# CESSProject/DeOSS

Measured on AMD Instinct MI355X. Metric: device-resident GiB/s hashed to Merkle root; 1/2/4/8 MI355X scaling, higher is better.
Workload: dtype u32; 1 GPU; BASELINE configs[1]: 1 object of 8 GiB (8589934592 B) in 1 chunk-range shard(s) of 8 GiB, chunk 33554432 B (256 leaves); object_bytes=8589934592, chunk=33554432, leaves=256, parallelism=single GPU

## Files before the change

### deoss_amd/csrc/merkle_capi.hip

```cpp
#include <hip/hip_runtime.h>
#include <rccl/rccl.h>

#include <algorithm>
#include <atomic>
#include <chrono>
#include <condition_variable>
#include <deque>
#include <cerrno>
#include <cstdarg>
#include <cstdlib>
#include <cstdio>
#include <cstring>
#include <functional>
#include <map>
#include <memory>
#include <future>
#include <mutex>
#include <string>
#include <thread>
#include <type_traits>
#include <vector>

#include "deoss_merkle.h"
#include "merkle_kernels.hpp"
// ... 200 lines not shown
                std::unique_lock<std::mutex> lk(mu);
                cv.wait(lk, [&] { return stop || !q.empty(); });
                if (q.empty()) return;
                it = q.front();
                q.pop_front();
                active++;
            }
            (void)hipSetDevice(it.dev);
            (void)hipGetLastError();
            if (it.pinned) host_release(it.p);
            else dev_release(it.dev, it.p);
            {
                std::lock_guard<std::mutex> lk(mu);
                active--;
            }
            idle.notify_all();
        }
    }
    void drain() {
        std::unique_lock<std::mutex> lk(mu);
        idle.wait(lk, [&] { return q.empty() && active == 0; });
    }
    void finish() {
        {
            std::lock_guard<std::mutex> lk(mu);
            stop = true;
        }
        cv.notify_one();
        if (th.joinable()) th.join();
    }
    ~Reaper() { finish(); }
};

void reaper_put(Reaper* r, int dev, void* p, bool pinned) { r->put(dev, p, pinned); }
void reaper_drain(Reaper* r) { r->drain(); }

void par_copy(const std::vector<dm_copy::CopyItem>& items) { dm_copy::CopyPool::get().run(items); }

struct StreamKit {
    static constexpr int kEvents = 10, kSlots = 4;
    hipStream_t copy = nullptr;
    hipStream_t code = nullptr, comp[2] = {nullptr, nullptr};
    hipEvent_t ev[kEvents] = {};
    PinnedBuf slot[kSlots];
    PinnedBuf tabs;
    uint64_t tabs_used = 0;
};

struct Dev {
    int id = 0;
    int cus = 256;
    hipStream_t stream = nullptr;
    hipStream_t copy = nullptr;
    DevBuf data, nodes_a, nodes_b, leaves, tab_addr, tab_len, tab_first, tab_ids, root, gather;
    DevBuf proof_paths, proof_bits, proof_roots;
    DevBuf aes_win;
    PinnedBuf stage[2];
    PinnedBuf htab;
    uint64_t htab_used = 0;
    hipEvent_t ev_done = nullptr;
    hipEvent_t ev_copy[2] = {nullptr, nullptr}, ev_step[2] = {nullptr, nullptr}, ev_htab = nullptr;
    bool has_last = false;
    hipEvent_t ev_tail = nullptr;
    hipStream_t tail_stream = nullptr;
    uint64_t keep_bytes = kLaneKeepBytes;
    std::vector<hipEvent_t> tev;
    size_t ntimed = 0;
};

}

struct DevSlot {
    std::mutex mu;
    std::atomic<int> load{0};
    std::mutex kit_mu;
    std::vector<StreamKit*> kits;
};

inline uint64_t next_ctx_serial() {
    static std::atomic<uint64_t> n{0};
    return ++n;
}

struct dm_ctx {
    std::vector<Dev> devs;
    int nphys = 1;
    int lanes = 1;
    std::unique_ptr<DevSlot[]> slots;
    std::atomic<uint32_t> rr{0};
    std::mutex route_mu;
    std::mutex comm_mu;
    std::map<int, std::vector<ncclComm_t>> comms;
    std::mutex err_mu;
    std::string err;
    Reaper reaper;
    bool timing = false;
    std::atomic<int> leaf_mode{DM_LEAF_AUTO};
    bool force_sharded = false;
    dm_plan::RouteConstants route_k;
    bool fail_comm_init = false;
    bool virtual_devs = false;
    bool shard_ok = true;
    const uint64_t serial = next_ctx_serial();
    bool keep_claimed = false;
    std::mutex xmu;
    uint64_t x_n = 0;
    double x_sum_us = 0, x_max_us = 0;
    int x_last_G = 0;
};

namespace {

thread_local std::string t_err;

int set_err(int code, const char* msg) {
    t_err = msg;
    return code;
}

int bad_arg() { return set_err(DM_ERR_INVALID, "invalid argument"); }

thread_local std::vector<int> t_call_devs;
thread_local int t_call_lane = -1;
thread_local uint64_t t_call_ctx = 0;

void note_call(const dm_ctx* c, int g, int G) {
    t_call_ctx = c->serial;
    t_call_devs.clear();
    if (G == 1) {
        t_call_devs.push_back(g % c->nphys);
        t_call_lane = g / c->nphys;
    } else {
        for (int i = 0; i < G; i++) t_call_devs.push_back(i);
        t_call_lane = 0;
    }
}

int fail(dm_ctx* c, int code, const char* fmt, ...) {
    char buf[1024];
    va_list ap;
    va_start(ap, fmt);
    vsnprintf(buf, sizeof buf, fmt, ap);
    va_end(ap);
    if (c) {
        std::lock_guard<std::mutex> lk(c->err_mu);
        c->err = buf;
    }
    t_err = buf;
    return code;
}

#define HIP_TRY(expr)                                                                         \
    do {                                                                                      \
        hipError_t e_ = (expr);                                                               \
        if (e_ != hipSuccess)                                                                 \
            return fail(c, e_ == hipErrorOutOfMemory ? DM_ERR_NOMEM : DM_ERR_HIP, "%s: %s (%s:%d)", \
                        #expr, hipGetErrorString(e_), __FILE__, __LINE__);                    \
    } while (0)

#define RC_TRY(expr)                 \
    do {                             \
        int rc_ = (expr);            \
        if (rc_ != DM_OK) return rc_; \
    } while (0)

#define NCCL_TRY(expr)                                                                         \
    do {                                                                                       \
        ncclResult_t r_ = (expr);                                                              \
        if (r_ != ncclSuccess)                                                                 \
            return fail(c, DM_ERR_RCCL, "%s: %s", #expr, ncclGetErrorString(r_));              \
    } while (0)

hipStream_t pick_stream(Dev&, void* s) { return static_cast<hipStream_t>(s); }

struct DeviceRestore {
    int prev = -1;
    DeviceRestore() {
        if (hipGetDevice(&prev) != hipSuccess) {
            prev = -1;
            (void)hipGetLastError();
        }
// ... 168 lines not shown
int device_of(dm_ctx* c, const void* p) {
    int phys = 0;
    if (c->nphys > 1 && p) {
        hipPointerAttribute_t attr{};
        if (hipPointerGetAttributes(&attr, p) == hipSuccess)
            for (int i = 0; i < c->nphys; i++)
                if (c->devs[i].id == attr.device) {
                    phys = i;
                    break;
                }
        (void)hipGetLastError();
    }
    std::lock_guard<std::mutex> lk(c->route_mu);
    return choose_lane(c, 0, phys);
}

int begin_call(dm_ctx* c, Dev& d, hipStream_t s) {
    HIP_TRY(hipSetDevice(d.id));
    if (d.has_last) HIP_TRY(hipStreamWaitEvent(s, d.ev_tail, 0));
    d.has_last = true;
    d.tail_stream = s;
    return DM_OK;
}

bool is_aligned16(const void* p) { return (reinterpret_cast<uintptr_t>(p) & 15) == 0; }

hipEvent_t* timing_record(dm_ctx* c, Dev& d) {
    if (!c->timing) return nullptr;
    const size_t need = 3 * (d.ntimed + 1);
    while (d.tev.size() < need) {
        hipEvent_t e = nullptr;
        if (hipEventCreate(&e) != hipSuccess) return nullptr;
        d.tev.push_back(e);
    }
    return &d.tev[3 * d.ntimed++];
}

int tables_begin(dm_ctx* c, Dev& d, uint64_t bytes) {
    HIP_TRY(hipEventSynchronize(d.ev_htab));
    HIP_TRY(d.htab.ensure(std::max<uint64_t>(round_up(bytes, 256) + 4096, 1ull << 20)));
    d.htab_used = 0;
    return DM_OK;
}

int upload(dm_ctx* c, Dev& d, hipStream_t s, DevBuf& dst, const void* src, uint64_t bytes) {
    HIP_TRY(dst.ensure(std::max<uint64_t>(bytes, 8)));
    if (bytes == 0) return DM_OK;
    if (d.htab_used + bytes > d.htab.cap) return fail(c, DM_ERR_INVALID, "table bounce buffer overflow");
    uint8_t* h = d.htab.u8() + d.htab_used;
    std::memcpy(h, src, bytes);
    d.htab_used = round_up(d.htab_used + bytes, 256);
    HIP_TRY(hipMemcpyAsync(dst.p, h, bytes, hipMemcpyHostToDevice, s));
    HIP_TRY(hipEventRecord(d.ev_htab, s));
    return DM_OK;
}

int reduce_stages(dm_ctx* c, Dev& d, hipStream_t s, const uint8_t* in, uint64_t m, uint32_t D, uint8_t* dst) {
    std::vector<uint32_t> ks;
    for (uint32_t r = D; r > 0;) {
        uint32_t k = std::min<uint32_t>(9, r);
        ks.push_back(k);
        r -= k;
    }
    HIP_TRY(d.nodes_a.ensure(std::max<uint64_t>(ceil_div(m, 2), 1) * 32));
    HIP_TRY(d.nodes_b.ensure(std::max<uint64_t>(ceil_div(m, 2), 1) * 32));
    const uint8_t* cur = in;
    for (size_t i = 0; i < ks.size(); i++) {
        uint8_t* out = (i + 1 == ks.size()) ? dst : (cur == d.nodes_a.u8() ? d.nodes_b.u8() : d.nodes_a.u8());
        const uint64_t grid = ceil_div(m, dm::kReduceTile);
        hipLaunchKernelGGL(dm::reduce_kernel, dim3((uint32_t)grid), dim3(dm::kBlock), 0, s, cur, m, ks[i], out);
        HIP_TRY(hipGetLastError());
        m = ceil_shift(m, ks[i]);
        cur = out;
    }
    return DM_OK;
}

int pick_leaf_kernel(const dm_ctx* c, const Dev& d, uint64_t n) {
    static_assert(dm_plan::kQuadLeaves == dm::kQuadLeaves && dm_plan::kLatLeaves == dm::kLatLeaves, "plan shapes");
    return dm_plan::leaf_kind(n, d.cus, c->leaf_mode.load());
}

template <bool TABLE, bool ALIGNED>
void launch_leaves_t(hipStream_t s, const dm::LeafArgs& la, int kind, int cus) {
    const uint64_t n = la.nleaves;
    const dim3 qgrid((uint32_t)ceil_div(n, dm::kQuadLeaves));
    if (kind == DM_LEAF_QUAD && qgrid.x > 2 * (uint64_t)cus) {
        hipLaunchKernelGGL(dm::quad_shape_primer, dim3(4 * (uint32_t)cus), dim3(dm::kLatThreads), dm::kQuadLdsBytes, s, 0);
        hipLaunchKernelGGL((dm::leaf_kernel_quad<TABLE, ALIGNED, true>), qgrid, dim3(dm::kLatThreads), 0, s, la);
    }
    else if (kind == DM_LEAF_QUAD)
        hipLaunchKernelGGL((dm::leaf_kernel_quad<TABLE, ALIGNED, false>), qgrid, dim3(dm::kLatThreads), 0, s, la);
    else if (kind == DM_LEAF_PAIR)
        hipLaunchKernelGGL((dm::leaf_kernel_pair<TABLE, ALIGNED>), dim3((uint32_t)ceil_div(n, dm::kPairLeaves)),
                           dim3(dm::kLatThreads), 0, s, la);
    else if (kind == DM_LEAF_LATENCY)
        hipLaunchKernelGGL((dm::leaf_kernel_lat<TABLE, ALIGNED>), dim3((uint32_t)ceil_div(n, dm::kLatLeaves)),
                           dim3(dm::kLatThreads), 0, s, la);
    else
        hipLaunchKernelGGL((dm::leaf_kernel<TABLE, ALIGNED>), dim3((uint32_t)ceil_div(n, dm::kBlock)), dim3(dm::kBlock),
                           0, s, la);
}

int launch_leaves(dm_ctx* c, const Dev& d, hipStream_t s, const dm::LeafArgs& la, bool table, bool aligned, int kind) {
    if (table) {
        if (aligned) launch_leaves_t<true, true>(s, la, kind, d.cus);
        else launch_leaves_t<true, false>(s, la, kind, d.cus);
    } else {
        if (aligned) launch_leaves_t<false, true>(s, la, kind, d.cus);
        else launch_leaves_t<false, false>(s, la, kind, d.cus);
    }
    HIP_TRY(hipGetLastError());
    return DM_OK;
}

int run_tree(dm_ctx* c, Dev& d, hipStream_t s, dm::LeafArgs la, bool table, bool aligned, int levels,
             uint8_t* dst, uint64_t* nout, uint8_t* leaf_dig) {
    const uint64_t n = la.nleaves;
    const int kind = pick_leaf_kernel(c, d, n);
    const uint32_t D = levels < 0 ? std::max<uint32_t>(1, ceil_log2(n)) : (uint32_t)levels;
    const uint32_t fuse_max = kind == DM_LEAF_QUAD ? dm::kQuadFuseMax
                              : kind == DM_LEAF_PAIR ? dm::kPairFuseMax
                              : kind == DM_LEAF_LATENCY ? dm::kLatFuseMax : dm::kLeafFuseMax;
    const uint32_t L1 = std::min<uint32_t>(fuse_max, D);
    const uint64_t m1 = ceil_shift(n, L1);
    la.byte_off = 0;
    la.byte_end = ~0ull;
    la.state = nullptr;
    la.fuse_levels = L1;
    uint8_t* k1_out = dst;
    if (D > L1) {
        HIP_TRY(d.leaves.ensure(m1 * 32));
        k1_out = d.leaves.u8();
    }
    if (L1 == 0) {
        la.digests = dst;
        la.level_out = nullptr;
    } else {
        la.digests = leaf_dig;
        la.level_out = k1_out;
    }
    hipEvent_t* tr = timing_record(c, d);
    if (tr) HIP_TRY(hipEventRecord(tr[0], s));
    RC_TRY(launch_leaves(c, d, s, la, table, aligned, kind));
    if (tr) HIP_TRY(hipEventRecord(tr[1], s));
    if (L1 == 0 && leaf_dig != nullptr && leaf_dig != dst)
        HIP_TRY(hipMemcpyAsync(leaf_dig, dst, n * 32, hipMemcpyDeviceToDevice, s));
    if (D > L1) RC_TRY(reduce_stages(c, d, s, k1_out, m1, D - L1, dst));
    if (tr) HIP_TRY(hipEventRecord(tr[2], s));
    *nout = ceil_shift(n, D);
    return DM_OK;
}

dm::LeafArgs uniform_args(const void* dev, uint64_t len, uint64_t chunk) {
    dm::LeafArgs la{};
    const uint64_t n = ceil_div(len, chunk);
    la.base = static_cast<const uint8_t*>(dev);
    la.pitch = chunk;
    la.leaf_len = chunk;
    la.last_len = len - (n - 1) * chunk;
    la.nleaves = n;
    return la;
}

dm::LeafArgs table_args(const void* addrs, const void* lens, uint64_t n, uint8_t* digests) {
    dm::LeafArgs la{};
    la.addrs = static_cast<const uint64_t*>(addrs);
    la.lens = static_cast<const uint64_t*>(lens);
    la.nleaves = n;
    la.byte_end = ~0ull;
    la.digests = digests;
    return la;
}

int table_args(dm_ctx* c, Dev& d, hipStream_t s, const uint64_t* addr, const uint64_t* lens, uint64_t n,
               uint64_t extra, dm::LeafArgs* la) {
    RC_TRY(tables_begin(c, d, n * 16 + extra));
    HIP_TRY(d.leaves.ensure(n * 32));
    RC_TRY(upload(c, d, s, d.tab_addr, addr, n * 8));
    RC_TRY(upload(c, d, s, d.tab_len, lens, n * 8));
    *la = table_args(d.tab_addr.p, d.tab_len.p, n, d.leaves.u8());
    return DM_OK;
}

int finish(dm_ctx* c, Dev& d, hipStream_t s, const uint8_t* nodes, uint64_t n, bool min_one, uint8_t* dst) {
    uint32_t D = ceil_log2(n);
    if (D == 0 && min_one) D = 1;
    if (D == 0) {
        HIP_TRY(hipMemcpyAsync(dst, nodes, 32, hipMemcpyDeviceToDevice, s));
        return DM_OK;
    }
    return reduce_stages(c, d, s, nodes, n, D, dst);
}
// ... 621 lines not shown
    return it == g_keep_claimed.end() ? 0 : it->second;
}

void keep_claim(int dev, int64_t delta) {
    std::lock_guard<std::mutex> lk(g_keep_mu);
    uint64_t& v = g_keep_claimed[dev];
    v = delta < 0 && (uint64_t)(-delta) > v ? 0 : v + delta;
}

uint64_t lane_keep_bytes() {
    const char* kb = std::getenv("DEOSS_LANE_KEEP_BYTES");
    if (!kb || !*kb) return kLaneKeepBytes;
    char* end = nullptr;
    const unsigned long long v = std::strtoull(kb, &end, 10);
    return (end != kb && *end == '\0' && kb[0] != '-') ? (uint64_t)v : kLaneKeepBytes;
}

int default_lanes(const int* devs, int ndev) {
    const char* v = std::getenv("DEOSS_LANES");
    if (v && *v) return std::min(std::max(std::atoi(v), 1), kMaxLanes);
    const uint64_t keep = std::max<uint64_t>(lane_keep_bytes(), 1);
    uint64_t lanes = 4;
    const int n = (devs && ndev > 0) ? ndev : 1;
    for (int i = 0; i < n; i++) {
        const int dev = (devs && ndev > 0) ? devs[i] : 0;
        size_t free_b = 0, total_b = 0;
        if (hipSetDevice(dev) != hipSuccess || hipMemGetInfo(&free_b, &total_b) != hipSuccess) {
            (void)hipGetLastError();
            continue;
        }
        const uint64_t by_free = (uint64_t)free_b / (2 * keep);
        const uint64_t half = (uint64_t)total_b / 2, claimed = keep_claimed(dev);
        const uint64_t by_budget = claimed >= half ? 0 : (half - claimed) / keep;
        lanes = std::min(lanes, std::max<uint64_t>(std::min(by_free, by_budget), 1));
    }
    return (int)lanes;
}

void no_sharding(dm_ctx* c, const char* why) {
    c->shard_ok = false;
    std::fprintf(stderr, "deoss_merkle: RCCL communicators over %d GPUs unavailable (%s); every call runs whole on "
                 "one GPU\n", c->nphys, why);
}

int ctx_create(dm_ctx** out, const int* devs, int ndev, int lanes, bool lanes_given) {
    if (!out || lanes < 1 || lanes > kMaxLanes) return bad_arg();
    *out = nullptr;
    DeviceRestore dev;
    int count = 0;
    if (hipGetDeviceCount(&count) != hipSuccess || count <= 0) return set_err(DM_ERR_NODEV, "no usable GPU");
    std::vector<int> ids;
    if (!devs || ndev <= 0) ids.push_back(0);
    else ids.assign(devs, devs + ndev);
    for (size_t i = 0; i < ids.size(); i++) {
        if (ids[i] < 0 || ids[i] >= count) return bad_arg();
        for (size_t j = 0; j < i; j++)
            if (ids[j] == ids[i]) return bad_arg();
    }
    const char* vd = std::getenv("DEOSS_VIRTUAL_DEVICES");
    const int nvirt = vd ? std::atoi(vd) : 0;
    if (nvirt > 1) {
        ids.assign((size_t)std::min(nvirt, 64), ids[0]);
        if (!lanes_given) lanes = 1;
    }
    dm_ctx* c = new dm_ctx();
    c->nphys = (int)ids.size();
    c->lanes = lanes;
    c->devs.resize(ids.size() * (size_t)lanes);
    c->slots.reset(new DevSlot[c->devs.size()]);
    const uint64_t keep = lane_keep_bytes();
    for (size_t i = 0; i < c->devs.size(); i++) {
        c->devs[i].id = ids[i % ids.size()];
        c->devs[i].keep_bytes = keep;
        int rc = init_device(c, c->devs[i]);
        if (rc != DM_OK) {
            dm_destroy(c);
            return rc;
        }
    }
    for (const Dev& d : c->devs) keep_claim(d.id, (int64_t)d.keep_bytes);
    c->keep_claimed = true;
    const char* fs = std::getenv("DEOSS_FORCE_SHARDED");
    c->force_sharded = fs != nullptr && fs[0] == '1';
    c->route_k = dm_plan::route_constants_from_env();
    c->virtual_devs = nvirt > 1;
    const char* tf = std::getenv("DEOSS_TEST_RCCL_INIT_FAIL");
    c->fail_comm_init = tf && tf[0] == '1' && ids.size() > 1 && !c->force_sharded;
    if ((ids.size() > 1 || c->force_sharded) && (!c->virtual_devs || c->fail_comm_init)) {
        std::vector<ncclComm_t>* cm = nullptr;
        const int rc = comms_for(c, (int)ids.size(), &cm);
        if (rc != DM_OK && c->force_sharded) {
            dm_destroy(c);
            return set_err(DM_ERR_RCCL, "ncclCommInitAll failed");
        }
        if (rc != DM_OK) {
            std::string why;
            {
                std::lock_guard<std::mutex> lk(c->err_mu);
                why.swap(c->err);
            }
            t_err.clear();
            no_sharding(c, why.c_str());
        }
    }
    *out = c;
    return DM_OK;
}

}

extern "C" {

int dm_create(dm_ctx** out, const int* devs, int ndev) {
    int first = (devs && ndev > 0) ? devs[0] : 0;
    int count = 0;
    DeviceRestore dr;
    if (hipGetDeviceCount(&count) != hipSuccess || count <= 0) return set_err(DM_ERR_NODEV, "no usable GPU");
    if (first < 0 || first >= count) return bad_arg();
    std::lock_guard<std::mutex> lk(g_create_mu);
    return ctx_create(out, devs, ndev, default_lanes(devs, ndev), false);
}

int dm_create_lanes(dm_ctx** out, const int* devs, int ndev, int lanes) {
    std::lock_guard<std::mutex> lk(g_create_mu);
    return ctx_create(out, devs, ndev, lanes, true);
}

int dm_can_shard(dm_ctx* ctx) { return ctx && ctx->nphys > 1 && (ctx->shard_ok || ctx->force_sharded) ? 1 : 0; }

int dm_keep_claimed(int hip_device, uint64_t* bytes) {
    if (!bytes || hip_device < 0) return bad_arg();
    *bytes = keep_claimed(hip_device);
    return DM_OK;
}

void dm_destroy(dm_ctx* ctx) {
    if (!ctx) return;
    DeviceRestore dev;
    for (auto& kv : ctx->comms)
        for (auto& cm : kv.second) (void)ncclCommDestroy(cm);
    for (size_t g = 0; g < ctx->devs.size() && ctx->slots; g++) {
        if (hipSetDevice(ctx->devs[g].id) != hipSuccess) continue;
        for (StreamKit* k : ctx->slots[g].kits) kit_destroy(k);
        ctx->slots[g].kits.clear();
    }
    ctx->reaper.finish();
    for (auto& d : ctx->devs) {
        if (ctx->keep_claimed) keep_claim(d.id, -(int64_t)d.keep_bytes);
        destroy_device(d);
    }
    delete ctx;
}

int dm_set_leaf_kernel(dm_ctx* ctx, int mode) {
    if (!ctx || mode < DM_LEAF_AUTO || mode > DM_LEAF_QUAD) return bad_arg();
    RangeLock lk(ctx);
    ctx->leaf_mode = mode;
    return DM_OK;
}

int dm_leaf_kernel_for(dm_ctx* ctx, uint64_t nleaves) {
    if (!ctx) return bad_arg();
    return pick_leaf_kernel(ctx, ctx->devs[0], nleaves);
}

int dm_set_timing(dm_ctx* ctx, int enable) {
// ... 286 lines not shown
```

### deoss_amd/csrc/merkle_kernels.hpp

```cpp
#pragma once
#include "quad_ring.hpp"
#include "sha256_gfx950.hpp"

namespace dm {

constexpr int kBlock = 256;
constexpr int kLeafFuseMax = 8;
constexpr int kReduceTile = 512;

struct LeafArgs {
    const uint8_t* base;
    uint64_t pitch;
    uint64_t leaf_len;
    uint64_t last_len;
    const uint64_t* addrs;
    const uint64_t* lens;
    uint64_t nleaves;
    uint64_t byte_off;
    uint64_t byte_end;
    uint32_t* state;
    uint8_t* digests;
    uint8_t* level_out;
    uint32_t fuse_levels;
};
// ... 642 lines not shown
        asm volatile(DM_QS_CONTQ DM_QS_BODYQ DM_QS_ENDTAILQ
                     : DM_QS_STATE, [h] "+v"(h), [g] "+v"(g)
                     : DM_QS_KIN);
    }
}

template <int G, int ROW, bool MIS, int K8 = 0>
__device__ __forceinline__ void quad_stage_blocks(uint32_t (&x)[4], uint32_t (&P)[4], uint32_t& h, uint32_t& g,
                                                  uint4 (&S)[3][4], const uint4* kw, uint3 sh, uint32_t msk) {
    __builtin_amdgcn_s_waitcnt(kLgkmWait0);
    if constexpr (K8 + 2 < kQuadBlocks) {
#pragma unroll
        for (int t = 0; t < 4; t++) S[(K8 + 2) % 3][t] = kw[(K8 + 2) * ROW + 4 * t * G];
    }
    quad_block_regs<MIS, K8>(x, P, h, g, S[K8 % 3], S[(K8 + 1) % 3][0], sh, msk);
    if constexpr (K8 + 1 < kQuadBlocks) quad_stage_blocks<G, ROW, MIS, K8 + 1>(x, P, h, g, S, kw, sh, msk);
}
template <int G, int ROW, bool MIS>
__device__ __forceinline__ void quad_stage_regs(uint32_t (&x)[4], const uint4* kw, uint3 sh, uint32_t msk) {
    uint4 S[3][4];
    uint32_t P[4] = {x[0], x[1], x[2], x[3]}, h, g;
#pragma unroll
    for (int k = 0; k < 2; k++) {
#pragma unroll
        for (int t = 0; t < 4; t++) S[k][t] = kw[k * ROW + 4 * t * G];
    }
    quad_stage_blocks<G, ROW, MIS>(x, P, h, g, S, kw, sh, msk);
}

constexpr int kQuadWideRing = quad_ring::kWideDepth;
constexpr int kQuadSets = quad_ring::kSets;
template <int G, int ROW, int K8, bool FILL, bool TAIL, bool LOAD>
__device__ __forceinline__ void quad_xstage_block(uint32_t (&x)[4], uint32_t (&P)[4], uint32_t& h, uint32_t& g,
                                                  uint4 (&S)[kQuadSets][4], const uint4* src, uint3 sh, uint32_t msk) {
    static_assert((LOAD || !quad_ring::block_prefetches(K8, true)) && (!TAIL || !quad_ring::block_links(K8, true)) &&
                      !(FILL && TAIL) && quad_ring::prefetch_of(K8).block == (K8 + quad_ring::kAhead) % kQuadBlocks,
                  "only the last stage of a run skips a load or drains: quad_ring.hpp");
    __builtin_amdgcn_s_waitcnt(kLgkmWait0);
    if constexpr (LOAD) {
        constexpr quad_ring::BlockRef pf = quad_ring::prefetch_of(K8);
#pragma unroll
        for (int t = 0; t < 4; t++) S[quad_ring::set_of(K8 + quad_ring::kAhead)][t] = src[pf.block * ROW + 4 * t * G];
    }
    quad_block_regs<false, FILL ? 0 : TAIL ? kQuadBlocks - 1 : 1>(x, P, h, g, S[quad_ring::set_of(K8)],
                                                                 S[quad_ring::set_of(K8 + 1)][0], sh, msk);
}
template <int G, int ROW>
__device__ __forceinline__ uint32_t quad_run_xstage(uint32_t (&x)[4], const uint4* colp, uint32_t slot, uint64_t n,
                                                    uint3 sh, uint32_t msk) {
    uint4 S[kQuadSets][4];
    uint32_t P[4] = {x[0], x[1], x[2], x[3]}, h, g;
    const uint4* cur = colp + slot * 16 * G;
#pragma unroll
    for (int k = 0; k < quad_ring::kAhead; k++) {
#pragma unroll
        for (int t = 0; t < 4; t++) S[k][t] = cur[k * ROW + 4 * t * G];
    }
    quad_xstage_block<G, ROW, 0, true, false, true>(x, P, h, g, S, cur, sh, msk);
    for (uint64_t s = 1; s < n; s++) {
        slot = quad_ring::next_slot(slot, kQuadWideRing);
        const uint4* nxt = colp + slot * 16 * G;
        quad_xstage_block<G, ROW, 1, false, false, true>(x, P, h, g, S, cur, sh, msk);
        quad_xstage_block<G, ROW, 2, false, false, true>(x, P, h, g, S, cur, sh, msk);
        quad_xstage_block<G, ROW, 3, false, false, true>(x, P, h, g, S, cur, sh, msk);
        quad_xstage_block<G, ROW, 4, false, false, true>(x, P, h, g, S, cur, sh, msk);
        quad_xstage_block<G, ROW, 5, false, false, true>(x, P, h, g, S, cur, sh, msk);
        quad_xstage_block<G, ROW, 6, false, false, true>(x, P, h, g, S, nxt, sh, msk);
        quad_xstage_block<G, ROW, 7, false, false, true>(x, P, h, g, S, nxt, sh, msk);
        __syncthreads();
        quad_xstage_block<G, ROW, 0, false, false, true>(x, P, h, g, S, nxt, sh, msk);
        cur = nxt;
    }
    quad_xstage_block<G, ROW, 1, false, false, true>(x, P, h, g, S, cur, sh, msk);
    quad_xstage_block<G, ROW, 2, false, false, true>(x, P, h, g, S, cur, sh, msk);
    quad_xstage_block<G, ROW, 3, false, false, true>(x, P, h, g, S, cur, sh, msk);
    quad_xstage_block<G, ROW, 4, false, false, true>(x, P, h, g, S, cur, sh, msk);
    quad_xstage_block<G, ROW, 5, false, false, true>(x, P, h, g, S, cur, sh, msk);
    quad_xstage_block<G, ROW, 6, false, false, false>(x, P, h, g, S, cur, sh, msk);
    quad_xstage_block<G, ROW, 7, false, true, false>(x, P, h, g, S, cur, sh, msk);
    __syncthreads();
    return quad_ring::next_slot(slot, kQuadWideRing);
}

template <bool ALIGNED, int G>
__device__ __forceinline__ void quad_produce_block(const LeafView& v, Blk& cur, uint64_t b, uint4* kw) {
    if (b >= v.nb) return;
    uint32_t w[16];
    block_words(cur, w);
    if (b + kQuadBlocks < v.nb) cur = load_block<ALIGNED>(v.p + 64 * (b + kQuadBlocks));
#pragma unroll
    for (int q = 0; q < 16; q++) {
        uint32_t u[4];
#pragma unroll
        for (int k = 0; k < 4; k++) {
            const int t = 4 * q + k;
            uint32_t wt;
            if (t < 16) {
                wt = w[t];
            } else {
                wt = ssig1(w[(t - 2) & 15]) + w[(t - 7) & 15] + ssig0(w[(t - 15) & 15]) + w[t & 15];
                w[t & 15] = wt;
            }
            u[k] = 0u - (kSha256K[t] + wt);
        }
        kw[q * G] = make_uint4(u[0], u[1], u[2], u[3]);
    }
}

template <bool TABLE, bool ALIGNED, bool COMPACT>
__global__ __launch_bounds__(kLatThreads) void leaf_kernel_quad(LeafArgs a) {
    constexpr int ROW = COMPACT ? kQuadRow : kQuadLeaves;
    constexpr int G = kQuadBlocks * ROW;
    constexpr int DEPTH = COMPACT ? kLatRing : kQuadWideRing;
    __shared__ uint4 ring[COMPACT ? 1 : 2][kLatRing][16][G];
    __shared__ uint32_t lds_a[kQuadLeaves][8];
    __shared__ uint32_t lds_b[kQuadLeaves / 2][8];
    static_assert(DEPTH * sizeof(ring[0][0]) <= sizeof(ring), "the ring's stages must fit its LDS");
    static_assert(COMPACT || (3 * sizeof(ring) > (160u << 10) && sizeof(ring) <= (64u << 10) &&
                              2 * (sizeof(ring) + sizeof(lds_a) + sizeof(lds_b)) <= (160u << 10)),
                  "the wide K1Q must stay at exactly two workgroups per CU (160 KiB of LDS)");
    const uint32_t lane = threadIdx.x & 63;
    const bool producer = __builtin_amdgcn_readfirstlane(threadIdx.x) < 64;
    const uint32_t c = lane >> 3;
    const uint32_t j = lane & 7;
    const uint64_t first = (uint64_t)blockIdx.x * kQuadLeaves;
    const uint64_t i = first + c;
    const LeafView v = leaf_view<TABLE>(a, i);
    const uint64_t NB = wave_max_u64(v.nb);
    const uint64_t NI = (NB + kQuadBlocks - 1) / kQuadBlocks;
    if (producer) {
        Blk cur;
        if (j < v.nb) cur = load_block<ALIGNED>(v.p + 64 * j);
        if constexpr (!COMPACT) {
            uint4* const kw0 = &ring[0][0][0][j * ROW + c];
            uint32_t slot = 0;
            for (uint64_t s = 0; s < quad_ring::stages_before_first_barrier(DEPTH); s++) {
                if (s < NI) quad_produce_block<ALIGNED, G>(v, cur, s * kQuadBlocks + j, kw0 + slot * 16 * G);
                slot = quad_ring::next_slot(slot, DEPTH);
            }
            __syncthreads();
            for (uint64_t it = 0; it < NI; it++) {
                const uint64_t s = quad_ring::stage_written_after_barrier(it, DEPTH);
                if (s < NI) quad_produce_block<ALIGNED, G>(v, cur, s * kQuadBlocks + j, kw0 + slot * 16 * G);
                slot = quad_ring::next_slot(slot, DEPTH);
                __syncthreads();
            }
        } else {
            for (uint64_t it = 0; it < NI; it++) {
                const uint64_t b = it * kQuadBlocks + j;
                if (b < v.nb) {
                    uint32_t w[16];
                    block_words(cur, w);
                    if (b + kQuadBlocks < v.nb) cur = load_block<ALIGNED>(v.p + 64 * (b + kQuadBlocks));
                    uint4* kw = &ring[0][it % kLatRing][0][j * ROW + c];
#pragma unroll
                    for (int q = 0; q < 16; q++) {
                        uint32_t u[4];
#pragma unroll
                        for (int k = 0; k < 4; k++) {
                            const int t = 4 * q + k;
                            uint32_t wt;
                            if (t < 16) {
                                wt = w[t];
                            } else {
                                wt = ssig1(w[(t - 2) & 15]) + w[(t - 7) & 15] + ssig0(w[(t - 15) & 15]) + w[t & 15];
                                w[t & 15] = wt;
                            }
                            u[k] = 0u - (kSha256K[t] + wt);
                        }
                        kw[q * G] = make_uint4(u[0], u[1], u[2], u[3]);
                    }
                }
// ... 6 lines not shown
        const uint32_t cq = 2 * (lane >> 4) + ((lane >> 2) & 1);
        const bool role_a = (lane >> 3) & 1;
        const uint32_t p = lane & 3;
        const uint64_t iq = first + cq;
        const LeafView vq = leaf_view<TABLE>(a, iq);
        const uint3 sh = make_uint3(role_a ? (p == 0 ? 2 : p == 1 ? 13 : 22) : (p == 0 ? 6 : p == 1 ? 11 : 25), 0, 0);
        const uint32_t msk = role_a ? 0u : ~0u;
        uint32_t st0[8];
        if (vq.active) load_or_init_state(a, iq, st0);
        else init_state(st0);
        uint32_t x[4];
#pragma unroll
        for (int k = 0; k < 4; k++) x[k] = role_a ? st0[(k + 2) & 3] : st0[4 + k];
        const uint4* col = &ring[0][0][0][cq];
        __syncthreads();
        uint32_t xf[4];
#pragma unroll
        for (int k = 0; k < 4; k++) xf[k] = x[k];
        const uint64_t NS = uniform_u64(NI);
        uint32_t wslot = 0;
        for (uint64_t it = 0; it < NS;) {
            const bool running = COMPACT ? vq.active && vq.nb > it * kQuadBlocks
                                         : quad_ring::leaf_running(vq.active, vq.nb, it);
            const uint64_t end = uniform_u64(wave_min_u64(COMPACT ? (running ? vq.nb / kQuadBlocks : NS)
                                                                  : quad_ring::leaf_run_end(running, vq.nb, NS)));
            if constexpr (COMPACT) {
                for (; it < end; it++) {
                    quad_stage_regs<G, ROW, COMPACT>(x, col + (it % kLatRing) * 16 * G + p * G, sh, msk);
                    __syncthreads();
                }
            } else if (it < end) {
                wslot = quad_run_xstage<G, ROW>(x, col + p * G, wslot, end - it, sh, msk);
                it = end;
            }
            if (running) {
#pragma unroll
                for (int k = 0; k < 4; k++) xf[k] = x[k];
            }
            if (it == NS) break;
            if (!__any(COMPACT ? vq.active && vq.nb > it * kQuadBlocks && vq.nb < (it + 1) * kQuadBlocks
                               : quad_ring::leaf_ends_inside(vq.active, vq.nb, it)))
                continue;
            const uint4* kw = col + (COMPACT ? (uint32_t)(it % kLatRing) : wslot) * 16 * G;
            const uint64_t b0 = it * kQuadBlocks;
            for (uint32_t k = 0; k < kQuadBlocks; k++) {
                const uint4* kb = kw + k * ROW;
                if (b0 + k < vq.nb)
                    quad_block_skewed<COMPACT>(x, [kb](int g) { return kb[g * G]; }, sh, msk);
            }
            if (vq.nb > b0) {
#pragma unroll
                for (int k = 0; k < 4; k++) xf[k] = x[k];
            }
            __syncthreads();
            it++;
            wslot = quad_ring::next_slot(wslot, DEPTH);
        }
        uint32_t st[8];
#pragma unroll
        for (int k = 0; k < 4; k++) {
            st[k] = __shfl(xf[(k + 2) & 3], (int)(lane + 8), 64);
            st[4 + k] = xf[k];
        }
        if (vq.active && !role_a && p == 0) {
            leaf_epilogue<ALIGNED>(a, iq, vq, st);
#pragma unroll
            for (int k = 0; k < 8; k++) lds_a[cq][k] = st[k];
        }
    }
    if (a.fuse_levels == 0) return;
    __syncthreads();
    const uint32_t cnt = (uint32_t)((a.nleaves - first) < kQuadLeaves ? (a.nleaves - first) : kQuadLeaves);
    uint32_t (*res)[8];
    const uint32_t out_cnt = lds_reduce(lds_a, lds_b, cnt, a.fuse_levels, &res);
    if (threadIdx.x < out_cnt) {
        uint32_t o8[8];
#pragma unroll
        for (int k = 0; k < 8; k++) o8[k] = res[threadIdx.x][k];
        const uint64_t o = (uint64_t)blockIdx.x * (kQuadLeaves >> a.fuse_levels) + threadIdx.x;
        store_digest(a.level_out + 32 * o, o8);
    }
}

__global__ __launch_bounds__(kLatThreads) void quad_shape_primer(int x) {
    extern __shared__ uint4 dyn[];
    if (x == 12345) dyn[threadIdx.x] = make_uint4(1, 1, 1, 1);
}

__global__ __launch_bounds__(kBlock) void reduce_kernel(const uint8_t* in, uint64_t m, uint32_t levels,
                                                         uint8_t* out) {
    __shared__ uint32_t lds_a[kBlock][8];
    __shared__ uint32_t lds_b[kBlock / 2][8];
    const uint64_t base = (uint64_t)blockIdx.x * kReduceTile;
    const uint32_t cnt = (uint32_t)((m - base) < kReduceTile ? (m - base) : kReduceTile);
    const uint32_t t = threadIdx.x;
    const uint32_t next = (cnt + 1) >> 1;
    if (t < next) {
        uint32_t L[8], R[8], o[8];
        const uint32_t ri = (2 * t + 1 < cnt) ? 2 * t + 1 : cnt - 1;
        load_digest(in + 32 * (base + 2 * t), L);
        load_digest(in + 32 * (base + ri), R);
        node_hash(L, R, o);
#pragma unroll
        for (int k = 0; k < 8; k++) lds_a[t][k] = o[k];
    }
    __syncthreads();
    uint32_t (*res)[8];
    const uint32_t out_cnt = lds_reduce(lds_a, lds_b, next, levels - 1, &res);
    if (t < out_cnt) {
        uint32_t v[8];
#pragma unroll
        for (int k = 0; k < 8; k++) v[k] = res[t][k];
        store_digest(out + 32 * ((uint64_t)blockIdx.x * (kReduceTile >> levels) + t), v);
    }
}

__global__ __launch_bounds__(kBlock) void batch_root_kernel(const uint8_t* leaves, const uint64_t* leaf_first,
                                                             const uint32_t* obj_ids, uint8_t* roots) {
    __shared__ uint32_t lds_a[kBlock][8];
    __shared__ uint32_t lds_b[kBlock / 2][8];
    const uint32_t o = obj_ids[blockIdx.x];
    const uint64_t base = leaf_first[o];
    const uint32_t cnt = (uint32_t)(leaf_first[o + 1] - base);
    const uint32_t t = threadIdx.x;
    const uint32_t next = (cnt + 1) >> 1;
    if (t < next) {
        uint32_t L[8], R[8], h[8];
        const uint32_t ri = (2 * t + 1 < cnt) ? 2 * t + 1 : cnt - 1;
        load_digest(leaves + 32 * (base + 2 * t), L);
        load_digest(leaves + 32 * (base + ri), R);
        node_hash(L, R, h);
#pragma unroll
        for (int k = 0; k < 8; k++) lds_a[t][k] = h[k];
    }
    __syncthreads();
    uint32_t levels = 0;
    for (uint32_t c = next; c > 1; c = (c + 1) >> 1) levels++;
    uint32_t (*res)[8];
    lds_reduce(lds_a, lds_b, next, levels, &res);
    if (t == 0) {
        uint32_t v[8];
#pragma unroll
        for (int k = 0; k < 8; k++) v[k] = res[0][k];
        store_digest(roots + 32 * (uint64_t)o, v);
    }
}

__device__ __forceinline__ uint64_t splitmix64(uint64_t z) {
    z += 0x9e3779b97f4a7c15ULL;
    z = (z ^ (z >> 30)) * 0xbf58476d1ce4e5b9ULL;
    z = (z ^ (z >> 27)) * 0x94d049bb133111ebULL;
    return z ^ (z >> 31);
}

__global__ __launch_bounds__(kBlock) void fill_splitmix_kernel(uint64_t* dst, uint64_t word0, uint64_t nwords,
                                                                uint64_t seed) {
    const uint64_t stride = (uint64_t)gridDim.x * kBlock * 2;
    for (uint64_t j = ((uint64_t)blockIdx.x * kBlock + threadIdx.x) * 2; j < nwords; j += stride) {
        if (j + 1 < nwords) {
            ulonglong2 v = make_ulonglong2(splitmix64(seed ^ (word0 + j)), splitmix64(seed ^ (word0 + j + 1)));
            *reinterpret_cast<ulonglong2*>(dst + j) = v;
        } else {
            dst[j] = splitmix64(seed ^ (word0 + j));
        }
    }
}
// ... 34 lines not shown
```

Measured before the change: 16.86 GiB/s.

## Add single-wave self-feeding quad leaf kernel as default for large grids

Adds a new SHA-256 leaf kernel in which one 64-thread wave both expands message schedules into an LDS ring and consumes them for the compression rounds. This replaces the producer/consumer split with block-level barriers used by the existing quad kernel. The intent is to cut __syncthreads overhead and cross-wave handoff latency, with LDS sized so that exactly four workgroups fit per CU. The cost is that producer and consumer work are serialized inside one wave, so less latency hiding comes from other waves; an env var keeps the old ring path and a primed variant available.

```diff
diff --git a/deoss_amd/csrc/merkle_capi.hip b/deoss_amd/csrc/merkle_capi.hip
--- a/deoss_amd/csrc/merkle_capi.hip
+++ b/deoss_amd/csrc/merkle_capi.hip
@@ -306,6 +306,8 @@
     return ++n;
 }
 
+enum { kQuadCompactSelf = 0, kQuadCompactRing = 1, kQuadCompactSelfPrimed = 2 };
+
 struct dm_ctx {
     std::vector<Dev> devs;
     int nphys = 1;
@@ -321,6 +323,7 @@
     bool timing = false;
     std::atomic<int> leaf_mode{DM_LEAF_AUTO};
     bool force_sharded = false;
+    int quad_compact = kQuadCompactSelf;
     dm_plan::RouteConstants route_k;
     bool fail_comm_init = false;
     bool virtual_devs = false;
@@ -655,10 +658,16 @@
 }
 
 template <bool TABLE, bool ALIGNED>
-void launch_leaves_t(hipStream_t s, const dm::LeafArgs& la, int kind, int cus) {
+void launch_leaves_t(hipStream_t s, const dm::LeafArgs& la, int kind, int cus, int compact) {
     const uint64_t n = la.nleaves;
     const dim3 qgrid((uint32_t)ceil_div(n, dm::kQuadLeaves));
-    if (kind == DM_LEAF_QUAD && qgrid.x > 2 * (uint64_t)cus) {
+    if (kind == DM_LEAF_QUAD && qgrid.x > 2 * (uint64_t)cus && compact != kQuadCompactRing) {
+        if (compact == kQuadCompactSelfPrimed)
+            hipLaunchKernelGGL(dm::quad_shape_primer, dim3(4 * (uint32_t)cus), dim3(dm::kQuadSelfThreads),
+                               dm::kQuadSelfLdsBytes, s, 0);
+        hipLaunchKernelGGL((dm::leaf_kernel_quad_self<TABLE, ALIGNED>), qgrid, dim3(dm::kQuadSelfThreads), 0, s, la);
+    }
+    else if (kind == DM_LEAF_QUAD && qgrid.x > 2 * (uint64_t)cus) {
         hipLaunchKernelGGL(dm::quad_shape_primer, dim3(4 * (uint32_t)cus), dim3(dm::kLatThreads), dm::kQuadLdsBytes, s, 0);
         hipLaunchKernelGGL((dm::leaf_kernel_quad<TABLE, ALIGNED, true>), qgrid, dim3(dm::kLatThreads), 0, s, la);
     }
@@ -677,11 +686,11 @@
 
 int launch_leaves(dm_ctx* c, const Dev& d, hipStream_t s, const dm::LeafArgs& la, bool table, bool aligned, int kind) {
     if (table) {
-        if (aligned) launch_leaves_t<true, true>(s, la, kind, d.cus);
-        else launch_leaves_t<true, false>(s, la, kind, d.cus);
+        if (aligned) launch_leaves_t<true, true>(s, la, kind, d.cus, c->quad_compact);
+        else launch_leaves_t<true, false>(s, la, kind, d.cus, c->quad_compact);
     } else {
-        if (aligned) launch_leaves_t<false, true>(s, la, kind, d.cus);
-        else launch_leaves_t<false, false>(s, la, kind, d.cus);
+        if (aligned) launch_leaves_t<false, true>(s, la, kind, d.cus, c->quad_compact);
+        else launch_leaves_t<false, false>(s, la, kind, d.cus, c->quad_compact);
     }
     HIP_TRY(hipGetLastError());
     return DM_OK;
@@ -1469,6 +1478,9 @@
     c->keep_claimed = true;
     const char* fs = std::getenv("DEOSS_FORCE_SHARDED");
     c->force_sharded = fs != nullptr && fs[0] == '1';
+    const char* qc = std::getenv("DEOSS_QUAD_COMPACT");
+    c->quad_compact = qc == nullptr ? kQuadCompactSelf : std::strcmp(qc, "ring") == 0 ? kQuadCompactRing
+                      : std::strcmp(qc, "primed") == 0 ? kQuadCompactSelfPrimed : kQuadCompactSelf;
     c->route_k = dm_plan::route_constants_from_env();
     c->virtual_devs = nvirt > 1;
     const char* tf = std::getenv("DEOSS_TEST_RCCL_INIT_FAIL");
diff --git a/deoss_amd/csrc/merkle_kernels.hpp b/deoss_amd/csrc/merkle_kernels.hpp
--- a/deoss_amd/csrc/merkle_kernels.hpp
+++ b/deoss_amd/csrc/merkle_kernels.hpp
@@ -748,12 +748,12 @@
     return quad_ring::next_slot(slot, kQuadWideRing);
 }
 
-template <bool ALIGNED, int G>
+template <bool ALIGNED, int G, bool LOAD_NEXT = true>
 __device__ __forceinline__ void quad_produce_block(const LeafView& v, Blk& cur, uint64_t b, uint4* kw) {
     if (b >= v.nb) return;
     uint32_t w[16];
     block_words(cur, w);
-    if (b + kQuadBlocks < v.nb) cur = load_block<ALIGNED>(v.p + 64 * (b + kQuadBlocks));
+    if (LOAD_NEXT && b + kQuadBlocks < v.nb) cur = load_block<ALIGNED>(v.p + 64 * (b + kQuadBlocks));
 #pragma unroll
     for (int q = 0; q < 16; q++) {
         uint32_t u[4];
@@ -926,6 +926,118 @@
     }
 }
 
+#ifndef DM_QUAD_SELF_MIS
+#define DM_QUAD_SELF_MIS 0
+#endif
+constexpr bool kQuadSelfMis = DM_QUAD_SELF_MIS != 0;
+constexpr int kQuadSelfThreads = 64;
+constexpr int kQuadSelfSlots = 2;
+constexpr size_t kQuadSelfLdsBytes = sizeof(uint4) * kQuadSelfSlots * 16 * kQuadBlocks * kQuadRow +
+                                     4 * 8 * kQuadLeaves + 4 * 8 * (kQuadLeaves / 2);
+static_assert(kQuadSelfLdsBytes > (32u << 10) && kQuadSelfLdsBytes <= (40u << 10) &&
+                  4 * kQuadSelfLdsBytes <= (160u << 10) && 5 * kQuadSelfLdsBytes > (160u << 10),
+              "the self-feeding K1Q must stay at exactly four workgroups (one wave per SIMD) per CU");
+
+__device__ __forceinline__ void wave_lds_order() {
+    asm volatile("s_waitcnt lgkmcnt(0)" ::: "memory");
+}
+
+template <bool ALIGNED, int G>
+__device__ __forceinline__ void quad_self_produce(const LeafView& v, Blk& cur, uint64_t b, uint4* kw) {
+    quad_produce_block<ALIGNED, G, false>(v, cur, b, kw);
+    wave_lds_order();
+    if (b + kQuadBlocks < v.nb) cur = load_block<ALIGNED>(v.p + 64 * (b + kQuadBlocks));
+}
+
+template <bool TABLE, bool ALIGNED>
+__global__ __launch_bounds__(kQuadSelfThreads) void leaf_kernel_quad_self(LeafArgs a) {
+    constexpr bool MIS = kQuadSelfMis;
+    constexpr int ROW = kQuadRow;
+    constexpr int G = kQuadBlocks * ROW;
+    __shared__ uint4 ring[kQuadSelfSlots][16][G];
+    __shared__ uint32_t lds_a[kQuadLeaves][8];
+    __shared__ uint32_t lds_b[kQuadLeaves / 2][8];
+    static_assert(sizeof(ring) + sizeof(lds_a) + sizeof(lds_b) == kQuadSelfLdsBytes, "LDS footprint");
+    const uint32_t lane = threadIdx.x;
+    const uint64_t first = (uint64_t)blockIdx.x * kQuadLeaves;
+    const uint32_t c = lane & 7;
+    const uint32_t j = lane >> 3;
+    const LeafView v = leaf_view<TABLE>(a, first + c);
+    const uint64_t NB = wave_max_u64(v.nb);
+    const uint64_t NS = uniform_u64((NB + kQuadBlocks - 1) / kQuadBlocks);
+    Blk cur;
+    if (j < v.nb) cur = load_block<ALIGNED>(v.p + 64 * j);
+    uint4* const kwp = &ring[0][0][j * ROW + c];
+    const uint32_t cq = 2 * (lane >> 4) + ((lane >> 2) & 1);
+    const bool role_a = (lane >> 3) & 1;
+    const uint32_t p = lane & 3;
+    const uint64_t iq = first + cq;
+    const LeafView vq = leaf_view<TABLE>(a, iq);
+    const uint3 sh = make_uint3(role_a ? (p == 0 ? 2 : p == 1 ? 13 : 22) : (p == 0 ? 6 : p == 1 ? 11 : 25), 0, 0);
+    const uint32_t msk = role_a ? 0u : ~0u;
+    uint32_t st0[8];
+    if (vq.active) load_or_init_state(a, iq, st0);
+    else init_state(st0);
+    uint32_t x[4];
+#pragma unroll
+    for (int k = 0; k < 4; k++) x[k] = role_a ? st0[(k + 2) & 3] : st0[4 + k];
+    const uint4* col = &ring[0][0][cq];
+    uint32_t xf[4];
+#pragma unroll
+    for (int k = 0; k < 4; k++) xf[k] = x[k];
+    for (uint64_t it = 0; it < NS;) {
+        const bool running = quad_ring::leaf_running(vq.active, vq.nb, it);
+        const uint64_t end = uniform_u64(wave_min_u64(quad_ring::leaf_run_end(running, vq.nb, NS)));
+        for (; it < end; it++) {
+            quad_self_produce<ALIGNED, G>(v, cur, it * kQuadBlocks + j, kwp);
+            quad_stage_regs<G, ROW, MIS>(x, col + p * G, sh, msk);
+            wave_lds_order();
+        }
+        if (running) {
+#pragma unroll
+            for (int k = 0; k < 4; k++) xf[k] = x[k];
+        }
+        if (it == NS) break;
+        if (!__any(quad_ring::leaf_ends_inside(vq.active, vq.nb, it))) continue;
+        quad_self_produce<ALIGNED, G>(v, cur, it * kQuadBlocks + j, kwp);
+        const uint64_t b0 = it * kQuadBlocks;
+        for (uint32_t k = 0; k < kQuadBlocks; k++) {
+            const uint4* kb = col + k * ROW;
+            if (b0 + k < vq.nb)
+                quad_block_skewed<MIS>(x, [kb](int g) { return kb[g * G]; }, sh, msk);
+        }
+        if (vq.nb > b0) {
+#pragma unroll
+            for (int k = 0; k < 4; k++) xf[k] = x[k];
+        }
+        wave_lds_order();
+        it++;
+    }
+    uint32_t st[8];
+#pragma unroll
+    for (int k = 0; k < 4; k++) {
+        st[k] = __shfl(xf[(k + 2) & 3], (int)(lane + 8), 64);
+        st[4 + k] = xf[k];
+    }
+    if (vq.active && !role_a && p == 0) {
+        leaf_epilogue<ALIGNED>(a, iq, vq, st);
+#pragma unroll
+        for (int k = 0; k < 8; k++) lds_a[cq][k] = st[k];
+    }
+    if (a.fuse_levels == 0) return;
+    __syncthreads();
+    const uint32_t cnt = (uint32_t)((a.nleaves - first) < kQuadLeaves ? (a.nleaves - first) : kQuadLeaves);
+    uint32_t (*res)[8];
+    const uint32_t out_cnt = lds_reduce(lds_a, lds_b, cnt, a.fuse_levels, &res);
+    if (threadIdx.x < out_cnt) {
+        uint32_t o8[8];
+#pragma unroll
+        for (int k = 0; k < 8; k++) o8[k] = res[threadIdx.x][k];
+        const uint64_t o = (uint64_t)blockIdx.x * (kQuadLeaves >> a.fuse_levels) + threadIdx.x;
+        store_digest(a.level_out + 32 * o, o8);
+    }
+}
+
 __global__ __launch_bounds__(kLatThreads) void quad_shape_primer(int x) {
     extern __shared__ uint4 dyn[];
     if (x == 12345) dyn[threadIdx.x] = make_uint4(1, 1, 1, 1);
```

Result: no change. 16.87 GiB/s (median of 5 runs) (+0.0%).
